# second-state/qwen3_asr_rs

Measured on AMD Instinct MI355X. Metric: audio-seconds/sec (RTFx) Qwen3-ASR-0.6B greedy, 30s clips, higher is better.
Workload: dtype bf16

## Files before the change

### include/q3asr.h

```cpp
#ifndef Q3ASR_H
#define Q3ASR_H

#include <stdint.h>

#ifdef __cplusplus
extern "C" {
#endif

typedef struct q3a_engine q3a_engine;

typedef struct q3a_opts {
  int32_t precise;
  int32_t max_new_tokens;
  int32_t use_graph;
  int32_t debug_taps;
  int32_t valu_attention;
  int32_t reserved[11];
} q3a_opts;

void q3a_opts_default(q3a_opts* o);

typedef struct q3a_dims {
  int32_t enc_d_model, enc_layers, enc_heads, enc_ffn, num_mel_bins, n_window, n_window_infer,
      conv_channels, enc_output_dim, max_source_positions;
// ... 110 lines not shown
int32_t q3a_load_audio(const char* path, int32_t target_sr, float** samples_out, int64_t* n_out);
int32_t q3a_resample(const float* in, int64_t n, int32_t sr_in, int32_t sr_out, float** samples_out, int64_t* n_out);
int32_t q3a_resample_rubato(const float* in, int64_t n, int32_t sr_in, int32_t sr_out, float** samples_out, int64_t* n_out);
void q3a_free(void* p);

typedef struct q3a_tokenizer q3a_tokenizer;
int32_t q3a_tokenizer_create(const char* tokenizer_json_path, q3a_tokenizer** out);
void q3a_tokenizer_destroy(q3a_tokenizer* t);
int32_t q3a_tokenizer_decode(const q3a_tokenizer* t, const int32_t* ids, int32_t n, int32_t skip_special, char* out,
                             int32_t cap, int32_t* len);
int32_t q3a_tokenizer_encode(const q3a_tokenizer* t, const char* text, int32_t* ids, int32_t cap, int32_t* n);
int32_t q3a_normalize_nfc(const char* utf8, char* out, int32_t cap, int32_t* len);

int32_t q3a_parse_asr_output(const char* raw, int32_t language_forced, char* language, int32_t language_cap, char* text,
                             int32_t text_cap);
int32_t q3a_capitalize_first(const char* s, char* out, int32_t cap);

int32_t q3a_debug_set(const char* key, int32_t value);

int32_t q3a_selftest_gemm(int32_t device, int32_t M, int32_t N, int32_t K, int32_t split, float* max_abs_err,
                          float* ref_abs_max);
int32_t q3a_selftest_gemm16(int32_t device, int32_t M, int32_t N, int32_t K, int32_t reps, float* max_abs_err,
                            float* ref_abs_max, float* avg_us_bf16, float* avg_us_f32);

#ifdef __cplusplus
}
#endif
#endif
```

### qwen3_asr_rs_amd/_lib.py

```python
from __future__ import annotations

import ctypes as C
import os

HERE = os.path.dirname(os.path.abspath(__file__))
LIB_PATH = os.environ.get("Q3A_LIB") or os.path.join(HERE, "lib", "libq3asr_hip.so")

SYMBOLS = [
    "q3a_opts_default", "q3a_device_count", "q3a_engine_create", "q3a_arena_bytes", "q3a_arena_pack", "q3a_engine_create_from_arena",
    "q3a_engine_destroy", "q3a_last_error", "q3a_get_dims", "q3a_weights_rounded", "q3a_num_frames", "q3a_num_audio_tokens",
    "q3a_build_prompt", "q3a_mel", "q3a_encode", "q3a_prefill", "q3a_decode_step", "q3a_set_next_tokens",
    "q3a_upload_pcm", "q3a_run_resident", "q3a_fetch_ids", "q3a_transcribe_batch", "q3a_transcribe_batch_ptrs", "q3a_io_timings_last", "q3a_stage_timings",
    "q3a_profile_decode_step", "q3a_profile_weight_stream", "q3a_measure_peaks", "q3a_debug_read", "q3a_debug_set", "q3a_selftest_gemm", "q3a_selftest_gemm16",
    "q3a_load_audio", "q3a_resample", "q3a_resample_rubato", "q3a_free", "q3a_tokenizer_create", "q3a_tokenizer_destroy",
    "q3a_tokenizer_decode", "q3a_tokenizer_encode", "q3a_normalize_nfc", "q3a_parse_asr_output", "q3a_capitalize_first",
    "q3a_group_create", "q3a_group_destroy", "q3a_group_size", "q3a_group_used_rccl", "q3a_group_last_error",
    "q3a_group_engine", "q3a_group_partition", "q3a_group_transcribe", "q3a_group_transcribe_ptrs", "q3a_group_startup_seconds",
]


class Peaks(C.Structure):
    _fields_ = [("hbm_read_gbps", C.c_double), ("hbm_copy_gbps", C.c_double), ("hbm_triad_gbps", C.c_double), ("hbm_read_bytes", C.c_double),
                ("mfma_bf16_tflops", C.c_double), ("gemm_m", C.c_int32), ("gemm_n", C.c_int32), ("gemm_k", C.c_int32), ("n_cu", C.c_int32),
                ("reps", C.c_int32), ("reserved", C.c_int32), ("mfma_bf16_tflops_random", C.c_double)]


class Opts(C.Structure):
    _fields_ = [("precise", C.c_int32), ("max_new_tokens", C.c_int32), ("use_graph", C.c_int32),
                ("debug_taps", C.c_int32), ("valu_attention", C.c_int32), ("reserved", C.c_int32 * 11)]


class DimsC(C.Structure):
    _fields_ = [(n, C.c_int32) for n in (
        "enc_d_model", "enc_layers", "enc_heads", "enc_ffn", "num_mel_bins", "n_window", "n_window_infer",
        "conv_channels", "enc_output_dim", "max_source_positions", "vocab_size", "hidden_size",
        "intermediate_size", "dec_layers", "num_q_heads", "num_kv_heads", "head_dim", "tie_word_embeddings",
# ... 44 lines not shown
        "q3a_weights_rounded": (i32, [P]),
        "q3a_num_frames": (i64, [i64]),
        "q3a_num_audio_tokens": (i32, [P, i64]),
        "q3a_build_prompt": (i32, [i32, i32p, i32, i32p, i32p]),
        "q3a_mel": (i32, [P, f32p, i64p, i32, f32p, i32p]),
        "q3a_encode": (i32, [P, f32p, i32p]),
        "q3a_prefill": (i32, [P, i32p, i32p, i32, f32p, i32p]),
        "q3a_decode_step": (i32, [P, i32p, u8p, f32p]),
        "q3a_set_next_tokens": (i32, [P, i32p, i32]),
        "q3a_upload_pcm": (i32, [P, f32p, i64p, i32]),
        "q3a_run_resident": (i32, [P, i32p, i32, i32, i32]),
        "q3a_fetch_ids": (i32, [P, i32p, i32, i32p]),
        "q3a_transcribe_batch": (i32, [P, f32p, i64p, i32, i32p, i32, i32, i32, i32p, i32, i32p]),
        "q3a_transcribe_batch_ptrs": (i32, [P, C.POINTER(P), i64p, i32, i32p, i32, i32, i32, i32p, i32, i32p]),
        "q3a_io_timings_last": (i32, [P, C.POINTER(IoTimings)]),
        "q3a_stage_timings": (i32, [P, C.POINTER(Timings)]),
        "q3a_profile_decode_step": (i32, [P, C.POINTER(KernelProfile)]),
        "q3a_profile_weight_stream": (i32, [P, i32, f32p, C.POINTER(C.c_double), i32p]),
        "q3a_measure_peaks": (i32, [i32, i32, C.POINTER(Peaks)]),
        "q3a_debug_read": (i32, [P, C.c_char_p, P, u64, C.POINTER(u64)]),
        "q3a_debug_set": (i32, [C.c_char_p, i32]),
        "q3a_selftest_gemm": (i32, [i32, i32, i32, i32, i32, f32p, f32p]),
        "q3a_selftest_gemm16": (i32, [i32, i32, i32, i32, i32, f32p, f32p, f32p, f32p]),
        "q3a_load_audio": (i32, [C.c_char_p, i32, C.POINTER(f32p), i64p]),
        "q3a_resample": (i32, [f32p, i64, i32, i32, C.POINTER(f32p), i64p]),
        "q3a_resample_rubato": (i32, [f32p, i64, i32, i32, C.POINTER(f32p), i64p]),
        "q3a_free": (None, [P]),
        "q3a_tokenizer_create": (i32, [C.c_char_p, C.POINTER(P)]),
        "q3a_tokenizer_destroy": (None, [P]),
        "q3a_tokenizer_decode": (i32, [P, i32p, i32, i32, C.c_char_p, i32, i32p]),
        "q3a_tokenizer_encode": (i32, [P, C.c_char_p, i32p, i32, i32p]),
        "q3a_parse_asr_output": (i32, [C.c_char_p, i32, C.c_char_p, i32, C.c_char_p, i32]),
        "q3a_capitalize_first": (i32, [C.c_char_p, C.c_char_p, i32]),
        "q3a_normalize_nfc": (i32, [C.c_char_p, C.c_char_p, i32, i32p]),
        "q3a_group_create": (i32, [C.c_char_p, i32, i32p, C.POINTER(Opts), C.POINTER(P)]),
        "q3a_group_destroy": (None, [P]),
        "q3a_group_size": (i32, [P]),
        "q3a_group_used_rccl": (i32, [P]),
        "q3a_group_startup_seconds": (i32, [P, C.POINTER(C.c_double)]),
        "q3a_group_last_error": (C.c_char_p, [P]),
        "q3a_group_engine": (P, [P, i32]),
        "q3a_group_partition": (None, [i32, i32, i32, i32p, i32p]),
        "q3a_group_transcribe": (i32, [P, f32p, i64p, i32, i32p, i32, i32, i32, i32p, i32, i32p]),
        "q3a_group_transcribe_ptrs": (i32, [P, C.POINTER(P), i64p, i32, i32p, i32, i32, i32, i32p, i32, i32p]),
    }
    for name, (res, args) in sig.items():
# ... 6 lines not shown
```

### qwen3_asr_rs_amd/csrc/engine.cpp

```cpp
#include <hip/hip_runtime.h>

#include <sched.h>

#include <algorithm>
#include <atomic>
#include <chrono>
#include <cmath>
#include <cstdio>
#include <cstring>
#include <map>
#include <memory>
#include <mutex>
#include <string>
#include <thread>
#include <vector>

#include "../../include/q3asr.h"
#include "kernels.h"
#include "model.h"

using namespace q3a;

namespace {

// ... 49 lines not shown
};

}

namespace q3a {
void set_thread_error(const std::string& msg) { g_last_error = msg; }
}
namespace q3a {
Knobs& knobs() {
  static Knobs k;
  static std::once_flag once;
  std::call_once(once, [] {
    auto env = [](const char* name, std::atomic<int>& dst) { if (const char* e = getenv(name)) dst.store(atoi(e)); };
    env("Q3A_GEMM256_MIN_TILES", k.gemm256_min_tiles);
    env("Q3A_GEMM256_PERSIST", k.gemm256_persist);
    env("Q3A_GEMM256_GROUP_M", k.gemm256_group_m);
    env("Q3A_DATTN_BATCHED_MIN_WGS", k.dattn_batched_min_wgs);
    env("Q3A_DECODE_GROUP", k.decode_group_size);
    env("Q3A_DECODE_PARALLEL", k.decode_parallel_groups);
    env("Q3A_FUSE_QKROPE", k.fuse_qkrope);
    env("Q3A_SKINNY_Q", k.skinny_q);
    env("Q3A_EOS_RUN_AHEAD", k.eos_run_ahead);
    env("Q3A_SKINNY_GLU_HP3", k.skinny_glu_hp3);
  });
  return k;
}
}

struct q3a_engine {
  Dims d;
  ArenaLayout L;
  q3a_opts opts{};
  int device = 0;
  hipStream_t stream = nullptr;
  uint8_t* arena = nullptr;
  bool own_arena = false;
  uint32_t arena_flags = 0;
  std::string err;

  DevBuf dft, filt_t, pos_emb, rope_cos, rope_sin;
  int rope_positions = 0;

  int B = 0;
  std::vector<int64_t> n_samples, pcm_off, mel_off;
  std::vector<int> n_frames, n_chunks, T, tok_off;
  int total_chunks = 0, total_T = 0, max_frames = 0;
  bool have_mel = false, have_enc = false, have_prefill = false;
  std::vector<int> P, seq_off;
  int total_P = 0, max_ctx = 0, max_new = 0;
  std::vector<AttnSeg> enc_segs_h;
  int enc_max_seg = 0;

  DevBuf pcm, d_pcm_off, d_n_samples, d_mel_off, d_n_frames, mel, gmax, d_chunk_utt, d_chunk_frame0;
  DevBuf conv1, conv2, conv3, conv3_rowmap, convout_rowmap;
  DevBuf enc_x, enc_ln, enc_qkv, enc_ctx, enc_ffn, enc_segs, audio_embeds;
  DevBuf ids, audio_rowmap, row_seq, row_pos, dec_segs, last_rows;
  DevBuf dec_x, dec_ln, dec_qkv, dec_ctx, dec_act, kcache, vcache;
  DevBuf x_dec, d_pos, next_tok, out_ids, step_count, done, s_ln, s_qkv, s_ctx, s_act, logits, forced_tok, part_val, part_idx;
  DevBuf attn_pm, attn_pl, attn_po;
  DevBuf nn_x, nn_ss;
  DevBuf rope_cur;
  DevBuf enc_ctx16, dec_ctx16;
  DevBuf dec_q16;
  int n_cu = 256;
  DevBuf n_done;
  int* host_prog = nullptr;
  int* host_prog_dev = nullptr;
  DevBuf zero_page;
  int part_stride = 0, attn_nsplit = 0;
  size_t kv_layer_elems = 0;

  int gsize = 32;
  int k_parallel_groups = 1, k_skinny_q = 1, k_dattn_batched_min_wgs = 128, k_skinny_glu_hp3 = 1;
  std::vector<hipStream_t> chain_streams;
  std::vector<hipEvent_t> join_ev;
  hipEvent_t fork_ev = nullptr;

  static constexpr size_t kGraphCacheMax = 16;
  std::vector<std::pair<std::string, hipGraphExec_t>> graph_cache;
  int pos_hi_ = 0, live_nsplit_ = 0;
  int min_P_ = 0;

  hipStream_t up_stream = nullptr;
  void* pin_p = nullptr;
  size_t pin_cap = 0;
  std::vector<hipEvent_t> up_ev;
  hipEvent_t up_t0 = nullptr, up_t1 = nullptr;
  q3a_io_timings io{};
  bool geom_valid = false;

  q3a_timings timings{};
// ... 9 lines not shown
  template <typename T> const T* w(uint64_t off) const { return reinterpret_cast<const T*>(arena + off); }
  const float* wf(uint64_t off) const { return w<float>(off); }
  const uint16_t* wh(uint64_t off) const { return w<uint16_t>(off); }

  static bool light_tap(const char* name) { return strcmp(name, "dec_last_hidden") == 0 || strcmp(name, "head_in") == 0; }
  void tap(const char* name, const void* ptr, size_t bytes) {
    if (!opts.debug_taps || bytes == 0 || (opts.debug_taps == 2 && !light_tap(name))) return;
    DevBuf& t = taps[name];
    t.ensure(bytes);
    tap_bytes[name] = bytes;
    HIPCHK(hipMemcpyAsync(t.p, ptr, bytes, hipMemcpyDeviceToDevice, stream));
  }
  void tap_act(const char* name, const void* ptr, size_t elems) {
    if (!opts.debug_taps || elems == 0 || opts.debug_taps == 2) return;
    if (precise()) return tap(name, ptr, elems * 4);
    DevBuf& t = taps[name];
    t.ensure(elems * 4);
    tap_bytes[name] = elems * 4;
    KCHK(launch_from_bf16((const uint16_t*)ptr, t.as<float>(), elems, stream));
  }

  void act_gemm(const DevBuf& x, int lda, const uint16_t* W, int M, int N, int K, const GemmEpilogue& ep, bool glu) {
    if (precise()) KCHK(launch_gemm(x.as<float>(), lda, W, M, N, K, ep, glu, true, stream));
    else KCHK(launch_gemm16(x.as<uint16_t>(), lda, W, M, N, K, ep, glu, stream));
  }
  void act_conv(const DevBuf& x, int imgs, int H, int Wd, int C, const uint16_t* W, int Cout, const GemmEpilogue& ep) {
    if (precise()) KCHK(launch_conv3x3s2_gemm(x.as<float>(), imgs, H, Wd, C, W, Cout, ep, true, stream));
    else KCHK(launch_conv3x3s2_gemm16(x.as<uint16_t>(), zero_page.as<uint16_t>(), imgs, H, Wd, C, W, Cout, ep, stream));
  }
  void act_out(GemmEpilogue& ep, const DevBuf& buf) const {
    if (precise()) ep.out = buf.as<float>(); else ep.out16 = buf.as<uint16_t>();
  }
  uint16_t* act16(const DevBuf& buf) const { return precise() ? nullptr : buf.as<uint16_t>(); }

  template <class F> void timed(int kclass, double bytes, F&& fn) {
    if (!prof) {
      fn();
      return;
    }
    ProfEvent pe{kclass, bytes, nullptr, nullptr};
    HIPCHK(hipEventCreate(&pe.a));
    HIPCHK(hipEventCreate(&pe.b));
    HIPCHK(hipEventRecord(pe.a, stream));
    fn();
    HIPCHK(hipEventRecord(pe.b, stream));
    prof->push_back(pe);
  }
// ... 10 lines not shown
    if (e != hipSuccess || n_dev == 0)
      fail("no HIP device available: libq3asr_hip has no CPU fallback (hipGetDeviceCount: " + std::string(hipGetErrorString(e)) + ")");
    if (dev < 0 || dev >= n_dev) fail("device index out of range");
    HIPCHK(hipSetDevice(dev));
    KCHK(skinny_init());
    (void)hipDeviceGetAttribute(&n_cu, hipDeviceAttributeMultiprocessorCount, dev);
    HIPCHK(hipStreamCreateWithFlags(&stream, hipStreamNonBlocking));
    for (auto& x : ev) HIPCHK(hipEventCreate(&x));
    HIPCHK(hipHostMalloc((void**)&host_prog, 64, hipHostMallocMapped));
    memset(host_prog, 0, 64);
    HIPCHK(hipHostGetDevicePointer((void**)&host_prog_dev, host_prog, 0));
    n_done.ensure(64);
  }

  void init_tables() {
    auto dftm = make_dft_matrix(400, 416);
    auto filt = make_mel_filterbank_T(d.n_mels, 400, 16000, 202);
    auto pe = make_sinusoid_rows(d.tokens_per_chunk(), d.enc_d);
    upload(dft, dftm, stream);
    upload(filt_t, filt, stream);
    upload(pos_emb, pe, stream);
    zero_page.ensure(256);
    HIPCHK(hipMemsetAsync(zero_page.p, 0, 256, stream));
    ensure_rope(8192);
    HIPCHK(hipStreamSynchronize(stream));
  }

  void ensure_rope(int n_pos) {
    if (n_pos <= rope_positions) return;
    int n = std::max(n_pos, 8192);
    std::vector<float> c, s;
    make_rope_tables(n, d.head_dim, d.rope_theta, c, s);
    HIPCHK(hipStreamSynchronize(stream));
    upload(rope_cos, c, stream);
    upload(rope_sin, s, stream);
    HIPCHK(hipStreamSynchronize(stream));
    rope_positions = n;
  }

  void check_arena_header() {
    ArenaHeader h;
    HIPCHK(hipMemcpy(&h, arena, sizeof(h), hipMemcpyDeviceToHost));
    if (h.magic != kArenaMagic || h.version != kArenaVersion) fail("weight arena: bad magic/version");
    if (h.total_bytes != L.total) fail("weight arena: size does not match config.json");
    arena_flags = h.flags;
  }
// ... 834 lines not shown
    for (int s = 0; s < B; ++s) {
      int n = std::min(sc[s], max_new), len = 0;
      for (; len < n; ++len) {
        int t = all[(size_t)s * max_new + len];
        if (!fixed_mode_ && (t == kEos0 || t == kEos1)) break;
      }
      out_lens[s] = len;
      for (int i = 0; i < std::min(len, stride); ++i) out[(size_t)s * stride + i] = all[(size_t)s * max_new + i];
    }
  }
  bool fixed_mode_ = false;
  bool head_logits_ = true;

  ~q3a_engine() {
    drop_graphs();
    for (auto cs : chain_streams) (void)hipStreamDestroy(cs);
    for (auto ce : join_ev) (void)hipEventDestroy(ce);
    if (fork_ev) (void)hipEventDestroy(fork_ev);
    DevBuf* bufs[] = {&dft, &filt_t, &pos_emb, &rope_cos, &rope_sin, &pcm, &d_pcm_off, &d_n_samples, &d_mel_off, &d_n_frames,
                      &mel, &gmax, &d_chunk_utt, &d_chunk_frame0, &conv1, &conv2, &conv3, &conv3_rowmap, &convout_rowmap,
                      &enc_x, &enc_ln, &enc_qkv, &enc_ctx, &enc_ffn, &enc_segs, &audio_embeds, &ids, &audio_rowmap, &row_seq,
                      &row_pos, &dec_segs, &last_rows, &dec_x, &dec_ln, &dec_qkv, &dec_ctx, &dec_act, &kcache, &vcache, &x_dec,
                      &d_pos, &next_tok, &out_ids, &step_count, &done, &s_ln, &s_qkv, &s_ctx, &s_act, &logits, &forced_tok, &part_val, &part_idx, &attn_pm, &attn_pl, &attn_po,
                      &enc_ctx16, &dec_ctx16, &dec_q16, &zero_page, &rope_cur, &nn_x, &nn_ss, &n_done};
    for (auto* b : bufs) b->release();
    for (auto& kv : taps) kv.second.release();
    if (own_arena && arena) (void)hipFree(arena);
    if (host_prog) (void)hipHostFree(host_prog);
    if (up_stream) { (void)hipStreamSynchronize(up_stream); (void)hipStreamDestroy(up_stream); }
    if (pin_p) (void)hipHostFree(pin_p);
    for (auto ue : up_ev) (void)hipEventDestroy(ue);
    if (up_t0) (void)hipEventDestroy(up_t0);
    if (up_t1) (void)hipEventDestroy(up_t1);
    for (auto& x : ev)
      if (x) (void)hipEventDestroy(x);
    if (stream) (void)hipStreamDestroy(stream);
  }
};

void q3a_engine::scatter_audio_rows() {
  KCHK(launch_scatter_rows(audio_embeds.as<float>(), audio_rowmap.as<int>(), total_T, d.hidden, dec_x.as<float>(), stream));
}

#define Q3A_TRY(e) try {
#define Q3A_CATCH(e)                                 \
  }                                                  \
  catch (const std::exception& ex) {                 \
// ... 385 lines not shown
  size_t n = e->tap_bytes[name];
  if (actual) *actual = n;
  if (dst) {
    if (bytes < n) fail("q3a_debug_read: destination too small");
    HIPCHK(hipStreamSynchronize(e->stream));
    HIPCHK(hipMemcpy(dst, it->second.p, n, hipMemcpyDeviceToHost));
  }
  Q3A_CATCH(e)
}

int32_t q3a_debug_set(const char* key, int32_t value) {
  if (!key) return 1;
  Knobs& kn = knobs();
  if (strcmp(key, "gemm256_min_tiles") == 0) { kn.gemm256_min_tiles = value; return 0; }
  if (strcmp(key, "gemm256_persist") == 0) { kn.gemm256_persist = value; return 0; }
  if (strcmp(key, "gemm256_group_m") == 0) { kn.gemm256_group_m = value; return 0; }
  if (strcmp(key, "dattn_batched_min_wgs") == 0) { kn.dattn_batched_min_wgs = value; return 0; }
  if (strcmp(key, "decode_group_size") == 0) { kn.decode_group_size = value; return 0; }
  if (strcmp(key, "decode_parallel_groups") == 0) { kn.decode_parallel_groups = value; return 0; }
  if (strcmp(key, "fuse_qkrope") == 0) { kn.fuse_qkrope = value; return 0; }
  if (strcmp(key, "skinny_q") == 0) { kn.skinny_q = value; return 0; }
  if (strcmp(key, "eos_run_ahead") == 0) { kn.eos_run_ahead = value; return 0; }
  if (strcmp(key, "skinny_glu_hp3") == 0) { kn.skinny_glu_hp3 = value; return 0; }
  g_last_error = std::string("q3a_debug_set: unknown key '") + key + "'";
  return 1;
}

int32_t q3a_selftest_gemm(int32_t device, int32_t M, int32_t N, int32_t K, int32_t split, float* max_abs_err,
                          float* ref_abs_max) {
  q3a_engine* e = nullptr;
  Q3A_TRY(e)
  int n_dev = 0;
  if (hipGetDeviceCount(&n_dev) != hipSuccess || n_dev == 0) fail("no HIP device available");
  HIPCHK(hipSetDevice(device));
  std::vector<float> X((size_t)M * K);
  std::vector<uint16_t> W((size_t)N * K);
  uint32_t st = 12345u;
  auto rnd = [&]() { st = st * 1664525u + 1013904223u; return ((st >> 8) & 0xffff) / 65536.0f - 0.5f; };
  for (auto& v : X) v = rnd();
  for (auto& v : W) { float f = rnd(); uint32_t u; memcpy(&u, &f, 4); v = (uint16_t)(u >> 16); }
  DevBuf dX, dW, dY, dR;
  dX.ensure(X.size() * 4); dW.ensure(W.size() * 2); dY.ensure((size_t)M * N * 4); dR.ensure((size_t)M * N * 4);
  HIPCHK(hipMemcpy(dX.p, X.data(), X.size() * 4, hipMemcpyHostToDevice));
  HIPCHK(hipMemcpy(dW.p, W.data(), W.size() * 2, hipMemcpyHostToDevice));
  GemmEpilogue ep; ep.out = dY.as<float>(); ep.ldo = N;
  KCHK(launch_gemm(dX.as<float>(), K, dW.as<uint16_t>(), M, N, K, ep, false, split != 0, nullptr));
// ... 107 lines not shown
    hipEvent_t a, b;
    HIPCHK(hipEventCreate(&a));
    HIPCHK(hipEventCreate(&b));
    float ms = 0.f;
    HIPCHK(hipEventRecord(a, nullptr));
    for (int r = 0; r < reps; ++r) KCHK(launch_gemm16(dX16.as<uint16_t>(), K, dW.as<uint16_t>(), M, N, K, ep, false, nullptr));
    HIPCHK(hipEventRecord(b, nullptr));
    HIPCHK(hipEventSynchronize(b));
    HIPCHK(hipEventElapsedTime(&ms, a, b));
    if (avg_us_bf16) *avg_us_bf16 = ms * 1000.f / reps;
    HIPCHK(hipEventRecord(a, nullptr));
    for (int r = 0; r < reps; ++r) KCHK(launch_gemm(dX.as<float>(), K, dW.as<uint16_t>(), M, N, K, ep, false, false, nullptr));
    HIPCHK(hipEventRecord(b, nullptr));
    HIPCHK(hipEventSynchronize(b));
    HIPCHK(hipEventElapsedTime(&ms, a, b));
    if (avg_us_f32) *avg_us_f32 = ms * 1000.f / reps;
    (void)hipEventDestroy(a);
    (void)hipEventDestroy(b);
  }
  dX.release(); dX16.release(); dW.release(); dY.release(); dR.release();
  Q3A_CATCH(e)
}

}
```

### qwen3_asr_rs_amd/csrc/k_gemm16.hip

```cpp
#include <stdlib.h>

#include <type_traits>

#include "dev.h"
#include "kernels.h"

namespace q3a {
namespace {

typedef const void __attribute__((address_space(1)))* gptr_t;
typedef void __attribute__((address_space(3)))* lptr_t;

struct DenseA16 {
  const uint16_t* x;
  int lda;
  __device__ __forceinline__ void init_row(int m, int M, int& s0, int& s1, int& s2) const {
    s0 = m < M ? m : M - 1;
    s1 = s2 = 0;
  }
  __device__ __forceinline__ const uint16_t* row_ptr(int s0, int, int, int k0) const { return x + (size_t)s0 * lda + k0; }
};

struct ConvA16 {
  const uint16_t* x;
// ... 458 lines not shown
    }
    float4 v = *reinterpret_cast<const float4*>(&red[row * BN + c4]);
#pragma unroll
    for (int w = 1; w < 4; ++w) {
      const float4 p = *reinterpret_cast<const float4*>(&red[(w * BM + row) * BN + c4]);
      v.x += p.x; v.y += p.y; v.z += p.z; v.w += p.w;
    }
    if (ep.bias) { v.x += b4.x; v.y += b4.y; v.z += b4.z; v.w += b4.w; }
    if (ep.addend) { v.x += a4.x; v.y += a4.y; v.z += a4.z; v.w += a4.w; }
    if (ep.act == 1) { v.x = gelu_fast(v.x); v.y = gelu_fast(v.y); v.z = gelu_fast(v.z); v.w = gelu_fast(v.w); }
    if (ep.resid) { v.x += r4.x; v.y += r4.y; v.z += r4.z; v.w += r4.w; }
    if (ep.out16) {
      uint2 pk;
      pk.x = pack_bf16x2(v.x, v.y);
      pk.y = pack_bf16x2(v.z, v.w);
      *reinterpret_cast<uint2*>(ep.out16 + (size_t)orow * ep.ldo + n) = pk;
    } else {
      *reinterpret_cast<float4*>(ep.out + (size_t)orow * ep.ldo + n) = v;
    }
  }
  Q3A_STAMP_AT(ep.stamp, blockIdx.x, 3);
}

template <int BM, int BN, int BK, bool GLU, class ALoader>
void launch16(const ALoader& A, const uint16_t* W, int M, int N, int K, const GemmEpilogue& ep, hipStream_t s) {
  const int tiles = ((M + BM - 1) / BM) * ((N + BN - 1) / BN);
  constexpr bool ring = std::is_same<ALoader, DenseA16>::value && BK == 64 && BM <= 64 && BN <= 64;
  if constexpr (ring) {
    if (tiles <= 512) {
      hipLaunchKernelGGL((gemm16_kernel<BM, BN, BK, GLU, ALoader, 4>), dim3(tiles), dim3(256), 0, s, A, W, M, N, K, ep);
      return;
    }
    if (tiles <= 768) {
      hipLaunchKernelGGL((gemm16_kernel<BM, BN, BK, GLU, ALoader, 3>), dim3(tiles), dim3(256), 0, s, A, W, M, N, K, ep);
      return;
    }
  }
  hipLaunchKernelGGL((gemm16_kernel<BM, BN, BK, GLU, ALoader, 2>), dim3(tiles), dim3(256), 0, s, A, W, M, N, K, ep);
}

inline long tiles_of(int M, int N, int bm, int bn) { return (long)((M + bm - 1) / bm) * ((N + bn - 1) / bn); }

template <int BK, bool GLU, class ALoader>
void launch_sized16(const ALoader& A, const uint16_t* W, int M, int N, int K, const GemmEpilogue& ep, hipStream_t s) {
  if (M <= 32) launch16<32, 64, BK, GLU>(A, W, M, N, K, ep, s);
  else if (tiles_of(M, N, 128, 128) >= 384) launch16<128, 128, BK, GLU>(A, W, M, N, K, ep, s);
// ... 25 lines not shown
  hipLaunchKernelGGL(from_bf16_kernel, dim3((unsigned)blocks), dim3(256), 0, s, x, y, n);
  return nullptr;
}

const char* launch_gemm16(const uint16_t* X, int lda, const uint16_t* W, int M, int N, int K, const GemmEpilogue& ep,
                          bool glu, hipStream_t s) {
  if (M <= 0) return nullptr;
  if (K % 32 != 0 || lda % 8 != 0) return "gemm16: K must be a multiple of 32 and lda of 8";
  if (K % 64 == 0 && !ep.part_val && gemm256_eligible(M, N, K)) return launch_gemm256(X, lda, W, M, N, K, ep, glu, s);
  return launch_gemm16_small(X, lda, W, M, N, K, ep, glu, s);
}

const char* launch_gemm16_small(const uint16_t* X, int lda, const uint16_t* W, int M, int N, int K, const GemmEpilogue& ep,
                                bool glu, hipStream_t s) {
  if (M <= 0) return nullptr;
  if (K % 32 != 0 || lda % 8 != 0) return "gemm16: K must be a multiple of 32 and lda of 8";
  if (glu && N % 32 != 0) return "gemm16: GLU needs N % 32 == 0";
  if (ep.part_val && (M > 32 || glu || N % 4 != 0 || ep.ldo % 4 != 0 || K % 64 != 0 || ep.rowmap || ep.part_stride < (N + 63) / 64))
    return "gemm16: argmax partials need M <= 32, 4 | N, 4 | ldo, 64 | K, no row map and part_stride >= ceil(N / 64)";
  DenseA16 A{X, lda};
  static const bool ksplit_on = [] { const char* e = getenv("Q3A_GEMM16_KSPLIT"); return !e || atoi(e) != 0; }();
  if (ksplit_on && !glu && !ep.part_val && tiles_of(M, N, 32, 64) < 384 && K >= 512 && K % 128 == 0 && N % 4 == 0 && ep.ldo % 4 == 0) {
    const int tiles = ((M + 31) / 32) * ((N + 31) / 32);
    if (K % 256 == 0) hipLaunchKernelGGL((gemm16k_kernel<32, 256, DenseA16, 2>), dim3(tiles), dim3(256), 0, s, A, W, M, N, K, ep);
    else hipLaunchKernelGGL((gemm16k_kernel<32, 128, DenseA16, 4>), dim3(tiles), dim3(256), 0, s, A, W, M, N, K, ep);
    return nullptr;
  }
  static const bool force_bk32 = [] { const char* e = getenv("Q3A_GEMM16_BK32"); return e && atoi(e) != 0; }();
  if (K % 64 == 0 && !force_bk32) {
    if (glu) launch_sized16<64, true>(A, W, M, N, K, ep, s); else launch_sized16<64, false>(A, W, M, N, K, ep, s);
  } else {
    if (glu) launch_sized16<32, true>(A, W, M, N, K, ep, s); else launch_sized16<32, false>(A, W, M, N, K, ep, s);
  }
  return nullptr;
}

const char* launch_to_bf16(const float* x, uint16_t* y, size_t n, hipStream_t s) {
  if (n == 0) return nullptr;
  if (n % 4 != 0) return "to_bf16: n must be a multiple of 4";
  size_t blocks = (n / 4 + 255) / 256;
  if (blocks > 4096) blocks = 4096;
  hipLaunchKernelGGL(to_bf16_kernel, dim3((unsigned)blocks), dim3(256), 0, s, x, y, n / 4);
  return nullptr;
}

const char* launch_conv3x3s2_gemm16(const uint16_t* X, const uint16_t* zero_page, int imgs, int H, int Wd, int C,
// ... 13 lines not shown
```

### qwen3_asr_rs_amd/csrc/kernels.h

```cpp
#pragma once
#include <hip/hip_runtime.h>
#include <stdint.h>

#include <atomic>

#ifndef Q3A_STAMP_FIELD
#ifdef Q3A_STAMP
#define Q3A_STAMP_FIELD unsigned long long* stamp = nullptr;
#else
#define Q3A_STAMP_FIELD
#endif
#endif

namespace q3a {

struct GemmEpilogue {
  float* out = nullptr;
  uint16_t* out16 = nullptr;
  int ldo = 0;
  const float* bias = nullptr;
  int act = 0;
  const float* resid = nullptr;
  const int* rowmap = nullptr;
  const float* addend = nullptr;
  int addend_period = 1;
  float* part_val = nullptr;
  int* part_idx = nullptr;
  int part_stride = 0;
  Q3A_STAMP_FIELD
};
const char* launch_gemm(const float* X, int lda, const uint16_t* W, int M, int N, int K, const GemmEpilogue& ep,
                        bool glu, bool split, hipStream_t s);
const char* launch_conv3x3s2_gemm(const float* X, int imgs, int H, int Wd, int C, const uint16_t* Wt, int Cout,
                                  const GemmEpilogue& ep, bool split, hipStream_t s);
void launch_gemm_ref(const float* X, const uint16_t* W, float* Y, int M, int N, int K, hipStream_t s);
const char* launch_gemm16(const uint16_t* X, int lda, const uint16_t* W, int M, int N, int K, const GemmEpilogue& ep,
                          bool glu, hipStream_t s);
const char* launch_conv3x3s2_gemm16(const uint16_t* X, const uint16_t* zero_page, int imgs, int H, int Wd, int C,
                                    const uint16_t* Wt, int Cout, const GemmEpilogue& ep, hipStream_t s);
bool gemm256_eligible(int M, int N, int K);
const char* launch_gemm16_small(const uint16_t* X, int lda, const uint16_t* W, int M, int N, int K, const GemmEpilogue& ep,
                                bool glu, hipStream_t s);
struct Knobs {
  std::atomic<int> gemm256_min_tiles{128};
  std::atomic<int> gemm256_persist{1};
  std::atomic<int> gemm256_group_m{0};
  std::atomic<int> dattn_batched_min_wgs{128};
  std::atomic<int> decode_group_size{0};
  std::atomic<int> decode_parallel_groups{1};
  std::atomic<int> fuse_qkrope{1};
  std::atomic<int> skinny_q{1};
  std::atomic<int> eos_run_ahead{1};
  std::atomic<int> skinny_glu_hp3{1};
};
Knobs& knobs();
const char* launch_gemm256(const uint16_t* X, int lda, const uint16_t* W, int M, int N, int K, const GemmEpilogue& ep,
                           bool glu, hipStream_t s);
const char* launch_conv3x3s2_gemm256(const uint16_t* X, const uint16_t* zero_page, int imgs, int H, int Wd, int C,
                                     const uint16_t* Wt, int Cout, const GemmEpilogue& ep, hipStream_t s);
const char* launch_to_bf16(const float* x, uint16_t* y, size_t n, hipStream_t s);
const char* launch_from_bf16(const uint16_t* x, float* y, size_t n, hipStream_t s);

struct MelBatch {
  const float* pcm;
  const int64_t* pcm_off;
  const int64_t* n_samples;
  const int64_t* mel_off;
  const int* n_frames;
  float* mel;
  unsigned* gmax_key;
};
const char* launch_mel(const MelBatch& mb, int B, int max_frames, const float* dft ,
                       const float* filt_t , hipStream_t s);

struct ChunkTable {
// ... 162 lines not shown
```

### qwen3_asr_rs_amd/engine.py

```python
from __future__ import annotations

import ctypes as C
import os
from dataclasses import dataclass
from typing import List, Optional, Sequence, Tuple

import numpy as np

from . import _lib

EOS_TOKEN_IDS = (151643, 151645)


class Q3aError(RuntimeError):
    pass


def _f32p(a: np.ndarray):
    return a.ctypes.data_as(C.POINTER(C.c_float))


def _i32p(a: np.ndarray):
    return a.ctypes.data_as(C.POINTER(C.c_int32))

# ... 253 lines not shown
def measure_peaks(device: int = 0, reps: int = 5) -> dict:
    lib = _lib.load()
    pk = _lib.Peaks()
    if lib.q3a_measure_peaks(device, reps, C.byref(pk)) != 0:
        raise RuntimeError("q3a_measure_peaks failed (no HIP device, or less than 2 GiB of free device memory)")
    return {"hbm_read_GBps": round(pk.hbm_read_gbps, 1), "hbm_copy_GBps": round(pk.hbm_copy_gbps, 1), "hbm_triad_GBps": round(pk.hbm_triad_gbps, 1),
            "mfma_bf16_TFLOPs": round(pk.mfma_bf16_tflops, 1), "mfma_bf16_TFLOPs_random_data": round(pk.mfma_bf16_tflops_random, 1), "gemm": [pk.gemm_m, pk.gemm_n, pk.gemm_k], "read_sweep_bytes": int(pk.hbm_read_bytes),
            "n_cu": pk.n_cu, "best_of": pk.reps}


def selftest_gemm16(M: int, N: int, K: int, reps: int = 0, device: int = 0) -> dict:
    lib = _lib.load()
    err, ref, t16, t32 = C.c_float(), C.c_float(), C.c_float(), C.c_float()
    rc = lib.q3a_selftest_gemm16(device, M, N, K, reps, C.byref(err), C.byref(ref), C.byref(t16), C.byref(t32))
    if rc != 0:
        raise Q3aError((lib.q3a_last_error(None) or b"").decode())
    flops = 2.0 * M * N * K
    out = {"err": err.value, "ref_max": ref.value}
    if reps > 0:
        out.update(us_bf16=t16.value, us_f32=t32.value, tflops_bf16=flops / t16.value / 1e6, tflops_f32=flops / t32.value / 1e6)
    return out


def selftest_gemm(M: int, N: int, K: int, split: bool = False, device: int = 0) -> Tuple[float, float]:
    lib = _lib.load()
    err, ref = C.c_float(), C.c_float()
    rc = lib.q3a_selftest_gemm(device, M, N, K, int(split), C.byref(err), C.byref(ref))
    if rc != 0:
        raise Q3aError((lib.q3a_last_error(None) or b"").decode())
    return err.value, ref.value


from .audio import AsrTokenizer, capitalize_first, load_audio, parse_asr_output


@dataclass
class TranscribeResult:
    text: str
    language: str
    raw_output: str
    ids: List[int]


class AsrInference:

    def __init__(self, engine: HipEngine, tokenizer=None):
# ... 27 lines not shown
```

Measured before the change: 476.2.

## Add split-K gemm16 kernel with atomic last-arriver reduction for small-tile GEMMs

Adds a split-K bf16 GEMM kernel for skinny or small GEMMs. Each output tile is split four ways along K across workgroups, partial fp32 tiles go to a global scratch slab, and the last arriving workgroup, found with an atomic counter, sums them and applies the epilogue. The goal is more parallelism when there are too few tiles to fill the CUs. The cost is extra scratch traffic, a counter-reset protocol that must stay correct under graph replay, and a different summation order. It is enabled by default through a knob and comes with a bit-exact selftest.

```diff
diff --git a/include/q3asr.h b/include/q3asr.h
--- a/include/q3asr.h
+++ b/include/q3asr.h
@@ -156,6 +156,7 @@
                           float* ref_abs_max);
 int32_t q3a_selftest_gemm16(int32_t device, int32_t M, int32_t N, int32_t K, int32_t reps, float* max_abs_err,
                             float* ref_abs_max, float* avg_us_bf16, float* avg_us_f32);
+int32_t q3a_selftest_gemm16_splitk(int32_t device, int32_t M, int32_t N, int32_t K, int32_t* mismatches, int32_t* counters_left);
 
 #ifdef __cplusplus
 }
diff --git a/qwen3_asr_rs_amd/_lib.py b/qwen3_asr_rs_amd/_lib.py
--- a/qwen3_asr_rs_amd/_lib.py
+++ b/qwen3_asr_rs_amd/_lib.py
@@ -11,7 +11,7 @@
     "q3a_engine_destroy", "q3a_last_error", "q3a_get_dims", "q3a_weights_rounded", "q3a_num_frames", "q3a_num_audio_tokens",
     "q3a_build_prompt", "q3a_mel", "q3a_encode", "q3a_prefill", "q3a_decode_step", "q3a_set_next_tokens",
     "q3a_upload_pcm", "q3a_run_resident", "q3a_fetch_ids", "q3a_transcribe_batch", "q3a_transcribe_batch_ptrs", "q3a_io_timings_last", "q3a_stage_timings",
-    "q3a_profile_decode_step", "q3a_profile_weight_stream", "q3a_measure_peaks", "q3a_debug_read", "q3a_debug_set", "q3a_selftest_gemm", "q3a_selftest_gemm16",
+    "q3a_profile_decode_step", "q3a_profile_weight_stream", "q3a_measure_peaks", "q3a_debug_read", "q3a_debug_set", "q3a_selftest_gemm", "q3a_selftest_gemm16", "q3a_selftest_gemm16_splitk",
     "q3a_load_audio", "q3a_resample", "q3a_resample_rubato", "q3a_free", "q3a_tokenizer_create", "q3a_tokenizer_destroy",
     "q3a_tokenizer_decode", "q3a_tokenizer_encode", "q3a_normalize_nfc", "q3a_parse_asr_output", "q3a_capitalize_first",
     "q3a_group_create", "q3a_group_destroy", "q3a_group_size", "q3a_group_used_rccl", "q3a_group_last_error",
@@ -102,6 +102,7 @@
         "q3a_debug_set": (i32, [C.c_char_p, i32]),
         "q3a_selftest_gemm": (i32, [i32, i32, i32, i32, i32, f32p, f32p]),
         "q3a_selftest_gemm16": (i32, [i32, i32, i32, i32, i32, f32p, f32p, f32p, f32p]),
+        "q3a_selftest_gemm16_splitk": (i32, [i32, i32, i32, i32, i32p, i32p]),
         "q3a_load_audio": (i32, [C.c_char_p, i32, C.POINTER(f32p), i64p]),
         "q3a_resample": (i32, [f32p, i64, i32, i32, C.POINTER(f32p), i64p]),
         "q3a_resample_rubato": (i32, [f32p, i64, i32, i32, C.POINTER(f32p), i64p]),
diff --git a/qwen3_asr_rs_amd/csrc/engine.cpp b/qwen3_asr_rs_amd/csrc/engine.cpp
--- a/qwen3_asr_rs_amd/csrc/engine.cpp
+++ b/qwen3_asr_rs_amd/csrc/engine.cpp
@@ -95,6 +95,7 @@
     env("Q3A_SKINNY_Q", k.skinny_q);
     env("Q3A_EOS_RUN_AHEAD", k.eos_run_ahead);
     env("Q3A_SKINNY_GLU_HP3", k.skinny_glu_hp3);
+    env("Q3A_GEMM16_SPLITK", k.gemm16_splitk);
   });
   return k;
 }
@@ -140,6 +141,8 @@
   int* host_prog = nullptr;
   int* host_prog_dev = nullptr;
   DevBuf zero_page;
+  static constexpr int kSplitKTiles = 384;
+  DevBuf splitk_part, splitk_cnt;
   int part_stride = 0, attn_nsplit = 0;
   size_t kv_layer_elems = 0;
 
@@ -195,7 +198,14 @@
 
   void act_gemm(const DevBuf& x, int lda, const uint16_t* W, int M, int N, int K, const GemmEpilogue& ep, bool glu) {
     if (precise()) KCHK(launch_gemm(x.as<float>(), lda, W, M, N, K, ep, glu, true, stream));
-    else KCHK(launch_gemm16(x.as<uint16_t>(), lda, W, M, N, K, ep, glu, stream));
+    else if (knobs().gemm16_splitk.load() == 0 || !splitk_part.p) KCHK(launch_gemm16(x.as<uint16_t>(), lda, W, M, N, K, ep, glu, stream));
+    else {
+      GemmEpilogue e = ep;
+      e.splitk_part = splitk_part.as<float>();
+      e.splitk_cnt = splitk_cnt.as<unsigned>();
+      e.splitk_tiles = kSplitKTiles;
+      KCHK(launch_gemm16(x.as<uint16_t>(), lda, W, M, N, K, e, glu, stream));
+    }
   }
   void act_conv(const DevBuf& x, int imgs, int H, int Wd, int C, const uint16_t* W, int Cout, const GemmEpilogue& ep) {
     if (precise()) KCHK(launch_conv3x3s2_gemm(x.as<float>(), imgs, H, Wd, C, W, Cout, ep, true, stream));
@@ -252,6 +262,11 @@
     upload(pos_emb, pe, stream);
     zero_page.ensure(256);
     HIPCHK(hipMemsetAsync(zero_page.p, 0, 256, stream));
+    if (!precise()) {
+      splitk_part.ensure((size_t)kSplitKTiles * 4 * 64 * 64 * 4);
+      splitk_cnt.ensure((size_t)kSplitKTiles * 64);
+      HIPCHK(hipMemsetAsync(splitk_cnt.p, 0, (size_t)kSplitKTiles * 64, stream));
+    }
     ensure_rope(8192);
     HIPCHK(hipStreamSynchronize(stream));
   }
@@ -1132,7 +1147,7 @@
                       &enc_x, &enc_ln, &enc_qkv, &enc_ctx, &enc_ffn, &enc_segs, &audio_embeds, &ids, &audio_rowmap, &row_seq,
                       &row_pos, &dec_segs, &last_rows, &dec_x, &dec_ln, &dec_qkv, &dec_ctx, &dec_act, &kcache, &vcache, &x_dec,
                       &d_pos, &next_tok, &out_ids, &step_count, &done, &s_ln, &s_qkv, &s_ctx, &s_act, &logits, &forced_tok, &part_val, &part_idx, &attn_pm, &attn_pl, &attn_po,
-                      &enc_ctx16, &dec_ctx16, &dec_q16, &zero_page, &rope_cur, &nn_x, &nn_ss, &n_done};
+                      &enc_ctx16, &dec_ctx16, &dec_q16, &zero_page, &splitk_part, &splitk_cnt, &rope_cur, &nn_x, &nn_ss, &n_done};
     for (auto* b : bufs) b->release();
     for (auto& kv : taps) kv.second.release();
     if (own_arena && arena) (void)hipFree(arena);
@@ -1564,6 +1579,7 @@
   if (strcmp(key, "skinny_q") == 0) { kn.skinny_q = value; return 0; }
   if (strcmp(key, "eos_run_ahead") == 0) { kn.eos_run_ahead = value; return 0; }
   if (strcmp(key, "skinny_glu_hp3") == 0) { kn.skinny_glu_hp3 = value; return 0; }
+  if (strcmp(key, "gemm16_splitk") == 0) { kn.gemm16_splitk = value; return 0; }
   g_last_error = std::string("q3a_debug_set: unknown key '") + key + "'";
   return 1;
 }
@@ -1717,4 +1733,104 @@
   Q3A_CATCH(e)
 }
 
-}
+int32_t q3a_selftest_gemm16_splitk(int32_t device, int32_t M, int32_t N, int32_t K, int32_t* mismatches, int32_t* counters_left) {
+  q3a_engine* e = nullptr;
+  Q3A_TRY(e)
+  int n_dev = 0;
+  if (hipGetDeviceCount(&n_dev) != hipSuccess || n_dev == 0) fail("no HIP device available");
+  HIPCHK(hipSetDevice(device));
+  if (M <= 0 || ((long)(M + 31) / 32) * ((N + 63) / 64) >= 384 || K < 512 || K % 256 != 0 || N % 4 != 0)
+    fail("selftest_gemm16_splitk: (M, N, K) does not take the split across workgroups");
+  const int tiles = ((M + 63) / 64) * ((N + 63) / 64);
+  const int P = 7;
+  uint32_t st = 4242u;
+  auto rnd = [&]() { st = st * 1664525u + 1013904223u; return ((st >> 8) & 0xffff) / 65536.0f - 0.5f; };
+  auto b16 = [](float f) { uint32_t u; memcpy(&u, &f, 4); return (uint16_t)(u >> 16); };
+  std::vector<uint16_t> X((size_t)M * K), W((size_t)N * K);
+  std::vector<float> bias(N), addend((size_t)P * N), resid((size_t)M * N);
+  std::vector<int> rowmap(M);
+  for (auto& v : X) v = b16(rnd());
+  for (auto& v : W) v = b16(rnd());
+  for (auto& v : bias) v = rnd();
+  for (auto& v : addend) v = rnd();
+  for (auto& v : resid) v = rnd();
+  for (int m = 0; m < M; ++m) rowmap[m] = (m % 11 == 5) ? -1 : M - 1 - m;
+  DevBuf dX, dW, dB, dA, dS, dM, dY, dPart, dCnt;
+  dX.ensure(X.size() * 2); dW.ensure(W.size() * 2); dB.ensure(bias.size() * 4); dA.ensure(addend.size() * 4);
+  dS.ensure(resid.size() * 4); dM.ensure(rowmap.size() * 4); dY.ensure(resid.size() * 4);
+  dPart.ensure((size_t)tiles * 4 * 64 * 64 * 4); dCnt.ensure((size_t)tiles * 64);
+  HIPCHK(hipMemcpy(dX.p, X.data(), X.size() * 2, hipMemcpyHostToDevice));
+  HIPCHK(hipMemcpy(dW.p, W.data(), W.size() * 2, hipMemcpyHostToDevice));
+  HIPCHK(hipMemcpy(dB.p, bias.data(), bias.size() * 4, hipMemcpyHostToDevice));
+  HIPCHK(hipMemcpy(dA.p, addend.data(), addend.size() * 4, hipMemcpyHostToDevice));
+  HIPCHK(hipMemcpy(dM.p, rowmap.data(), rowmap.size() * 4, hipMemcpyHostToDevice));
+  HIPCHK(hipMemset(dCnt.p, 0, (size_t)tiles * 64));
+  hipStream_t s = nullptr;
+  HIPCHK(hipStreamCreateWithFlags(&s, hipStreamNonBlocking));
+  int32_t mis = 0, left = 0;
+  const size_t bytes = resid.size() * 4;
+  std::vector<uint8_t> ref(bytes), got(bytes);
+  std::vector<unsigned> cnt((size_t)tiles * 16);
+  auto run = [&](GemmEpilogue ep, bool split, bool alias, std::vector<uint8_t>& out, hipGraphExec_t* capture) {
+    HIPCHK(hipMemsetAsync(dY.p, 0, bytes, s));
+    if (alias) HIPCHK(hipMemcpyAsync(dY.p, resid.data(), bytes, hipMemcpyHostToDevice, s));
+    if (split) { ep.splitk_part = dPart.as<float>(); ep.splitk_cnt = dCnt.as<unsigned>(); ep.splitk_tiles = tiles; }
+    if (capture) {
+      hipGraph_t g = nullptr;
+      HIPCHK(hipStreamBeginCapture(s, hipStreamCaptureModeThreadLocal));
+      KCHK(launch_gemm16(dX.as<uint16_t>(), K, dW.as<uint16_t>(), M, N, K, ep, false, s));
+      HIPCHK(hipStreamEndCapture(s, &g));
+      HIPCHK(hipGraphInstantiate(capture, g, nullptr, nullptr, 0));
+      HIPCHK(hipGraphDestroy(g));
+    } else {
+      KCHK(launch_gemm16(dX.as<uint16_t>(), K, dW.as<uint16_t>(), M, N, K, ep, false, s));
+    }
+    HIPCHK(hipStreamSynchronize(s));
+    HIPCHK(hipMemcpy(out.data(), dY.p, bytes, hipMemcpyDeviceToHost));
+  };
+  auto compare = [&](size_t n_bytes) {
+    for (size_t i = 0; i < n_bytes; i += 2) mis += memcmp(&ref[i], &got[i], 2) != 0;
+    HIPCHK(hipMemcpy(cnt.data(), dCnt.p, cnt.size() * 4, hipMemcpyDeviceToHost));
+    for (int t = 0; t < tiles; ++t) left += cnt[(size_t)t * 16] != 0;
+  };
+  HIPCHK(hipMemcpy(dS.p, resid.data(), bytes, hipMemcpyHostToDevice));
+  for (int c = 0; c < 3; ++c) {
+    GemmEpilogue ep;
+    ep.ldo = N;
+    size_t n_bytes = bytes;
+    bool alias = false;
+    if (c == 0) {
+      ep.out = dY.as<float>(); ep.bias = dB.as<float>(); ep.addend = dA.as<float>(); ep.addend_period = P;
+      ep.rowmap = dM.as<int>(); ep.resid = dS.as<float>();
+    } else if (c == 1) {
+      ep.out = dY.as<float>(); ep.resid = dY.as<float>(); ep.bias = dB.as<float>();
+      alias = true;
+    } else {
+      ep.out16 = dY.as<uint16_t>(); ep.bias = dB.as<float>(); ep.act = 1;
+      n_bytes = (size_t)M * N * 2;
+    }
+    run(ep, false, alias, ref, nullptr);
+    run(ep, true, alias, got, nullptr);
+    compare(n_bytes);
+    if (c == 0) {
+      hipGraphExec_t ge = nullptr;
+      run(ep, true, false, got, &ge);
+      for (int r = 0; r < 2; ++r) {
+        HIPCHK(hipMemsetAsync(dY.p, 0, bytes, s));
+        HIPCHK(hipGraphLaunch(ge, s));
+        HIPCHK(hipStreamSynchronize(s));
+        HIPCHK(hipMemcpy(got.data(), dY.p, bytes, hipMemcpyDeviceToHost));
+        compare(n_bytes);
+      }
+      HIPCHK(hipGraphExecDestroy(ge));
+    }
+  }
+  HIPCHK(hipStreamDestroy(s));
+  if (mismatches) *mismatches = mis;
+  if (counters_left) *counters_left = left;
+  dX.release(); dW.release(); dB.release(); dA.release(); dS.release(); dM.release(); dY.release();
+  dPart.release(); dCnt.release();
+  Q3A_CATCH(e)
+}
+
+}
diff --git a/qwen3_asr_rs_amd/csrc/k_gemm16.hip b/qwen3_asr_rs_amd/csrc/k_gemm16.hip
--- a/qwen3_asr_rs_amd/csrc/k_gemm16.hip
+++ b/qwen3_asr_rs_amd/csrc/k_gemm16.hip
@@ -504,6 +504,190 @@
   Q3A_STAMP_AT(ep.stamp, blockIdx.x, 3);
 }
 
+constexpr int kSplitS = 4;
+constexpr int kSplitCntStride = 16;
+
+template <int BKT>
+__global__ __launch_bounds__(256) void gemm16s_kernel(DenseA16 A, const uint16_t* __restrict__ Wt, int M, int N, int K,
+                                                      GemmEpilogue ep, float* part, unsigned* cnt) {
+  constexpr int BM = 64, BN = 64, BK = BKT / kSplitS, NS = 4;
+  constexpr int CPR = BK / 8;
+  constexpr int RPI = 64 / CPR;
+  constexpr int A_LOADS = BM / (4 * RPI);
+  constexpr int W_LOADS = BN / (4 * RPI);
+  constexpr int MI = 2, NI = 2;
+  constexpr int STAGE = (BM + BN) * BK;
+  constexpr int LDT = BN + 4;
+  static_assert(A_LOADS >= 1 && W_LOADS >= 1, "tile shape");
+  static_assert(NS * STAGE * 2 >= (BM * LDT + 4) * 4, "fp32 tile + arrival word must fit in the stages");
+  __shared__ __attribute__((aligned(16))) uint16_t lds[NS * STAGE];
+  Q3A_STAMP_AT(ep.stamp, blockIdx.x, 0);
+
+  const int tiles_m = (M + BM - 1) / BM, tiles_n = (N + BN - 1) / BN;
+  const int nwg = tiles_m * tiles_n * kSplitS;
+  int bid = blockIdx.x;
+  {
+    const int q = nwg / 8, r = nwg % 8, xcd = bid % 8, loc = bid / 8;
+    bid = (xcd < r ? xcd * (q + 1) : r * (q + 1) + (xcd - r) * q) + loc;
+  }
+  const int tile = bid / kSplitS, s = bid % kSplitS;
+  const int tm = tile % tiles_m, tn = tile / tiles_m;
+  const int m0 = tm * BM, n0 = tn * BN;
+  const int tid = threadIdx.x, lane = tid & 63, wave = tid >> 6;
+  const int wr = wave >> 1, wc = wave & 1;
+
+  const int l_row = lane / CPR, l_chunk = lane % CPR;
+  int a_s0[A_LOADS], a_s1[A_LOADS], a_s2[A_LOADS], a_src_chunk[A_LOADS];
+  const uint16_t* w_src[W_LOADS];
+#pragma unroll
+  for (int i = 0; i < A_LOADS; ++i) {
+    const int row = (i * 4 + wave) * RPI + l_row;
+    a_src_chunk[i] = l_chunk ^ swz<BK>(row);
+    A.init_row(m0 + row, M, a_s0[i], a_s1[i], a_s2[i]);
+  }
+#pragma unroll
+  for (int i = 0; i < W_LOADS; ++i) {
+    const int row = (i * 4 + wave) * RPI + l_row;
+    const int n = n0 + row;
+    w_src[i] = Wt + (size_t)(n < N ? n : N - 1) * K + s * BK + (l_chunk ^ swz<BK>(row)) * 8;
+  }
+  f32x4_t acc[MI][NI];
+#pragma unroll
+  for (int i = 0; i < MI; ++i)
+#pragma unroll
+    for (int j = 0; j < NI; ++j) acc[i][j] = f32x4_t{0.f, 0.f, 0.f, 0.f};
+
+  const int frag_row = lane & 15, frag_kc = lane >> 4;
+  const int KT = K / BKT;
+  auto issue_tile = [&](int kt, int buf) {
+    const int k0 = kt * BKT + s * BK;
+#pragma unroll
+    for (int i = 0; i < A_LOADS; ++i) {
+      const uint16_t* ap = A.row_ptr(a_s0[i], a_s1[i], a_s2[i], k0) + a_src_chunk[i] * 8;
+      __builtin_amdgcn_global_load_lds((gptr_t)ap, (lptr_t)(lds + buf * STAGE + (i * 4 + wave) * RPI * BK), 16, 0, 0);
+    }
+#pragma unroll
+    for (int i = 0; i < W_LOADS; ++i)
+      __builtin_amdgcn_global_load_lds((gptr_t)(w_src[i] + kt * BKT), (lptr_t)(lds + buf * STAGE + BM * BK + (i * 4 + wave) * RPI * BK),
+                                       16, 0, 0);
+  };
+#pragma unroll
+  for (int t = 0; t < NS - 1; ++t)
+    if (t < KT) issue_tile(t, t);
+  for (int kt = 0; kt < KT; ++kt) {
+    const int buf = kt % NS;
+    constexpr int L = A_LOADS + W_LOADS;
+    const int later = KT - 1 - kt;
+    if (later >= 2) g16_wait_vm<2 * L>();
+    else if (later == 1) g16_wait_vm<L>();
+    else g16_wait_vm<0>();
+    asm volatile("s_barrier" ::: "memory");
+    if (kt + NS - 1 < KT) issue_tile(kt + NS - 1, (kt + NS - 1) % NS);
+    if (kt == 0) Q3A_STAMP_AT(ep.stamp, blockIdx.x, 1);
+    const uint16_t* as = lds + buf * STAGE;
+    const uint16_t* ws = as + BM * BK;
+#pragma unroll
+    for (int ks = 0; ks < BK / 32; ++ks) {
+      bf16x8_t bfrag[NI];
+#pragma unroll
+      for (int j = 0; j < NI; ++j) {
+        const int row = wc * (BN / 2) + j * 16 + frag_row;
+        bfrag[j] = *reinterpret_cast<const bf16x8_t*>(&ws[row * BK + (((ks * 4 + frag_kc) ^ swz<BK>(row)) * 8)]);
+      }
+#pragma unroll
+      for (int i = 0; i < MI; ++i) {
+        const int row = wr * (BM / 2) + i * 16 + frag_row;
+        const bf16x8_t af = *reinterpret_cast<const bf16x8_t*>(&as[row * BK + (((ks * 4 + frag_kc) ^ swz<BK>(row)) * 8)]);
+#pragma unroll
+        for (int j = 0; j < NI; ++j) acc[i][j] = __builtin_amdgcn_mfma_f32_16x16x32_bf16(af, bfrag[j], acc[i][j], 0, 0, 0);
+      }
+    }
+  }
+  Q3A_STAMP_AT(ep.stamp, blockIdx.x, 2);
+
+  __syncthreads();
+  float* tl = reinterpret_cast<float*>(lds);
+  int* last_word = reinterpret_cast<int*>(lds) + BM * LDT;
+  {
+    const int col_in = lane & 15, row_in = (lane >> 4) * 4;
+#pragma unroll
+    for (int i = 0; i < MI; ++i)
+#pragma unroll
+      for (int j = 0; j < NI; ++j)
+#pragma unroll
+        for (int r = 0; r < 4; ++r) tl[(wr * 32 + i * 16 + row_in + r) * LDT + wc * 32 + j * 16 + col_in] = acc[i][j][r];
+  }
+  __syncthreads();
+  constexpr int NIT = BM * BN / 4 / 256;
+  typedef __attribute__((ext_vector_type(4))) unsigned u32x4;
+  const __amdgpu_buffer_rsrc_t slabs = __builtin_amdgcn_make_buffer_rsrc(part + (size_t)tile * kSplitS * BM * BN, 0, kSplitS * BM * BN * 4, 0x00020000);
+  constexpr int kSc1 = 16;
+#pragma unroll
+  for (int it = 0; it < NIT; ++it) {
+    const int e = tid + it * 256, row = e >> 4, c4 = (e & 15) * 4;
+    const float4 v = *reinterpret_cast<const float4*>(&tl[row * LDT + c4]);
+    const u32x4 u = {__float_as_uint(v.x), __float_as_uint(v.y), __float_as_uint(v.z), __float_as_uint(v.w)};
+    __builtin_amdgcn_raw_buffer_store_b128(u, slabs, (s * BM * BN + e * 4) * 4, 0, kSc1);
+  }
+  asm volatile("s_waitcnt vmcnt(0)" ::: "memory");
+  __syncthreads();
+  if (tid == 0) {
+    typedef unsigned __attribute__((address_space(1))) gu32;
+    gu32* c = (gu32*)(cnt + (size_t)tile * kSplitCntStride);
+    const unsigned t = __hip_atomic_fetch_add(c, 1u, __ATOMIC_RELAXED, __HIP_MEMORY_SCOPE_AGENT);
+    const int last = t == kSplitS - 1;
+    if (last) __hip_atomic_store(c, 0u, __ATOMIC_RELAXED, __HIP_MEMORY_SCOPE_AGENT);
+    *last_word = last;
+  }
+  __syncthreads();
+  if (!*last_word) return;
+  __builtin_amdgcn_fence(__ATOMIC_ACQUIRE, "wavefront");
+
+  int orow[NIT];
+#pragma unroll
+  for (int it = 0; it < NIT; ++it) {
+    const int e = tid + it * 256, row = e >> 4;
+    const int mc = m0 + row < M ? m0 + row : M - 1;
+    orow[it] = ep.rowmap ? ep.rowmap[mc] : mc;
+  }
+  float4 q[NIT][kSplitS], b4[NIT], a4[NIT], r4[NIT];
+#pragma unroll
+  for (int it = 0; it < NIT; ++it) {
+    const int e = tid + it * 256, row = e >> 4, c4 = (e & 15) * 4;
+    const int mc = m0 + row < M ? m0 + row : M - 1, nc = n0 + c4 < N ? n0 + c4 : 0;
+#pragma unroll
+    for (int t = 0; t < kSplitS; ++t) {
+      const u32x4 u = __builtin_amdgcn_raw_buffer_load_b128(slabs, (t * BM * BN + e * 4) * 4, 0, kSc1);
+      q[it][t] = make_float4(__uint_as_float(u.x), __uint_as_float(u.y), __uint_as_float(u.z), __uint_as_float(u.w));
+    }
+    if (ep.bias) b4[it] = *reinterpret_cast<const float4*>(ep.bias + nc);
+    if (ep.addend) a4[it] = *reinterpret_cast<const float4*>(ep.addend + (size_t)(mc % ep.addend_period) * ep.ldo + nc);
+    if (ep.resid) r4[it] = *reinterpret_cast<const float4*>(ep.resid + (size_t)(orow[it] < 0 ? 0 : orow[it]) * ep.ldo + nc);
+  }
+#pragma unroll
+  for (int it = 0; it < NIT; ++it) {
+    const int e = tid + it * 256, row = e >> 4, c4 = (e & 15) * 4;
+    const int m = m0 + row, n = n0 + c4;
+    if (m >= M || n >= N || orow[it] < 0) continue;
+    float4 v = q[it][0];
+#pragma unroll
+    for (int t = 1; t < kSplitS; ++t) { v.x += q[it][t].x; v.y += q[it][t].y; v.z += q[it][t].z; v.w += q[it][t].w; }
+    if (ep.bias) { v.x += b4[it].x; v.y += b4[it].y; v.z += b4[it].z; v.w += b4[it].w; }
+    if (ep.addend) { v.x += a4[it].x; v.y += a4[it].y; v.z += a4[it].z; v.w += a4[it].w; }
+    if (ep.act == 1) { v.x = gelu_fast(v.x); v.y = gelu_fast(v.y); v.z = gelu_fast(v.z); v.w = gelu_fast(v.w); }
+    if (ep.resid) { v.x += r4[it].x; v.y += r4[it].y; v.z += r4[it].z; v.w += r4[it].w; }
+    if (ep.out16) {
+      uint2 pk;
+      pk.x = pack_bf16x2(v.x, v.y);
+      pk.y = pack_bf16x2(v.z, v.w);
+      *reinterpret_cast<uint2*>(ep.out16 + (size_t)orow[it] * ep.ldo + n) = pk;
+    } else {
+      *reinterpret_cast<float4*>(ep.out + (size_t)orow[it] * ep.ldo + n) = v;
+    }
+  }
+  Q3A_STAMP_AT(ep.stamp, blockIdx.x, 3);
+}
+
 template <int BM, int BN, int BK, bool GLU, class ALoader>
 void launch16(const ALoader& A, const uint16_t* W, int M, int N, int K, const GemmEpilogue& ep, hipStream_t s) {
   const int tiles = ((M + BM - 1) / BM) * ((N + BN - 1) / BN);
@@ -575,6 +759,12 @@
   static const bool ksplit_on = [] { const char* e = getenv("Q3A_GEMM16_KSPLIT"); return !e || atoi(e) != 0; }();
   if (ksplit_on && !glu && !ep.part_val && tiles_of(M, N, 32, 64) < 384 && K >= 512 && K % 128 == 0 && N % 4 == 0 && ep.ldo % 4 == 0) {
     const int tiles = ((M + 31) / 32) * ((N + 31) / 32);
+    const long tiles64 = tiles_of(M, N, 64, 64);
+    if (K % 256 == 0 && ep.splitk_part && ep.splitk_cnt && tiles64 <= ep.splitk_tiles) {
+      hipLaunchKernelGGL((gemm16s_kernel<256>), dim3((unsigned)(tiles64 * kSplitS)), dim3(256), 0, s, A, W, M, N, K, ep, ep.splitk_part,
+                         ep.splitk_cnt);
+      return nullptr;
+    }
     if (K % 256 == 0) hipLaunchKernelGGL((gemm16k_kernel<32, 256, DenseA16, 2>), dim3(tiles), dim3(256), 0, s, A, W, M, N, K, ep);
     else hipLaunchKernelGGL((gemm16k_kernel<32, 128, DenseA16, 4>), dim3(tiles), dim3(256), 0, s, A, W, M, N, K, ep);
     return nullptr;
diff --git a/qwen3_asr_rs_amd/csrc/kernels.h b/qwen3_asr_rs_amd/csrc/kernels.h
--- a/qwen3_asr_rs_amd/csrc/kernels.h
+++ b/qwen3_asr_rs_amd/csrc/kernels.h
@@ -27,6 +27,9 @@
   float* part_val = nullptr;
   int* part_idx = nullptr;
   int part_stride = 0;
+  float* splitk_part = nullptr;
+  unsigned* splitk_cnt = nullptr;
+  int splitk_tiles = 0;
   Q3A_STAMP_FIELD
 };
 const char* launch_gemm(const float* X, int lda, const uint16_t* W, int M, int N, int K, const GemmEpilogue& ep,
@@ -51,6 +54,7 @@
   std::atomic<int> fuse_qkrope{1};
   std::atomic<int> skinny_q{1};
   std::atomic<int> eos_run_ahead{1};
+  std::atomic<int> gemm16_splitk{1};
   std::atomic<int> skinny_glu_hp3{1};
 };
 Knobs& knobs();
diff --git a/qwen3_asr_rs_amd/engine.py b/qwen3_asr_rs_amd/engine.py
--- a/qwen3_asr_rs_amd/engine.py
+++ b/qwen3_asr_rs_amd/engine.py
@@ -299,6 +299,15 @@
     return out
 
 
+def selftest_gemm16_splitk(M: int, N: int, K: int, device: int = 0) -> Tuple[int, int]:
+    lib = _lib.load()
+    mis, left = C.c_int32(), C.c_int32()
+    rc = lib.q3a_selftest_gemm16_splitk(device, M, N, K, C.byref(mis), C.byref(left))
+    if rc != 0:
+        raise Q3aError((lib.q3a_last_error(None) or b"").decode())
+    return mis.value, left.value
+
+
 def selftest_gemm(M: int, N: int, K: int, split: bool = False, device: int = 0) -> Tuple[float, float]:
     lib = _lib.load()
     err, ref = C.c_float(), C.c_float()
```

Result: no change. 477.3, median of 6 (+0.2%).
